# BatsResearch/menghini-neurips23-code

Measured on AMD Instinct MI355X. Metric: images/sec CLIP ViT-B/16 encode+prompt-step, higher is better.
Workload: dtype f16

## Files before the change

menghini-neurips23-code_amd/csrc/attention_split.hip:

```cpp
#include <math.h>

#include "common.h"

__device__ __forceinline__ int vt_index_fwd_s(int key, int d) { return vt_index(key, ((d >> 2) & 3) * 16 + (d >> 4) * 4 + (d & 3)); }

__device__ __forceinline__ void split8(const f32x4 a, const f32x4 b, half8& hi, half8& lo) {
    half4 h0, l0, h1, l1;
    split_f16x4(a, h0, l0);
    split_f16x4(b, h1, l1);
    hi = (half8){h0[0], h0[1], h0[2], h0[3], h1[0], h1[1], h1[2], h1[3]};
    lo = (half8){l0[0], l0[1], l0[2], l0[3], l1[0], l1[1], l1[2], l1[3]};
}

template <int KVC, bool CAUSAL, int NW>
__global__ __launch_bounds__(NW * 64) void attn_fwd_split_kernel(const float* __restrict__ qkv, half_t* __restrict__ out, int S, int H) {
    constexpr int SP = KVC * 32;
    constexpr float LOG2E = 1.4426950408889634f;
    constexpr float INV = 1.0f / (float)GRIP_SPLIT_LO_SCALE;
    extern __shared__ __attribute__((aligned(16))) char smem[];
    half_t* Kh = (half_t*)smem;
    half_t* Kl = Kh + SP * 64;
    half_t* Vh = Kl + SP * 64;
    half_t* Vl = Vh + SP * 64;

    const int tid = threadIdx.x, lane = tid & 63, wave = tid >> 6;
    const int D = H * 64;
    const int b = blockIdx.x / H, h = blockIdx.x - b * H;
    const size_t ld = (size_t)3 * D;
    const float* base = qkv + (size_t)b * S * ld + h * 64;
    const int li = lane & 15, lg = lane >> 4;
    const int n_qt = (S + 15) >> 4;

    for (int idx = tid; idx < SP * 8; idx += NW * 64) {
        const int row = idx >> 3, chunk = idx & 7;
        f32x4 a = {0.f, 0.f, 0.f, 0.f}, c = {0.f, 0.f, 0.f, 0.f};
        if (row < S) {
            const f32x4* p = (const f32x4*)(base + (size_t)row * ld + D + chunk * 8);
            a = p[0];
            c = p[1];
        }
        half8 hi, lo;
        split8(a, c, hi, lo);
        const int o = row * 64 + ((chunk ^ (row & 7)) * 8);
        *(half8*)(Kh + o) = hi;
        *(half8*)(Kl + o) = lo;
    }
    for (int idx = tid; idx < ((SP / 2 + 31) / 32) * 256; idx += NW * 64) {
        const int lane_rp = idx & 31, chunk = ((idx >> 5) & 1) + 2 * ((idx >> 6) & 3), rblk = idx >> 8;
        const int r0 = 2 * (rblk * 32 + lane_rp);
        if (r0 >= SP) continue;
        f32x4 z = {0.f, 0.f, 0.f, 0.f};
        f32x4 a0 = z, a1 = z, b0 = z, b1 = z;
        if (r0 < S) { const f32x4* p = (const f32x4*)(base + (size_t)r0 * ld + 2 * D + chunk * 8); a0 = p[0]; a1 = p[1]; }
        if (r0 + 1 < S) { const f32x4* p = (const f32x4*)(base + (size_t)(r0 + 1) * ld + 2 * D + chunk * 8); b0 = p[0]; b1 = p[1]; }
        half8 h0, l0, h1, l1;
        split8(a0, a1, h0, l0);
        split8(b0, b1, h1, l1);
#pragma unroll
        for (int j = 0; j < 8; ++j) {
            const int o = vt_index_fwd_s(r0, chunk * 8 + j);
            *(half2v*)(Vh + o) = (half2v){h0[j], h1[j]};
            *(half2v*)(Vl + o) = (half2v){l0[j], l1[j]};
        }
    }
    __syncthreads();

    for (int qt = wave; qt < n_qt; qt += NW) {
        asm volatile("" ::: "memory");
        const int qrow = qt * 16 + li;
        const int qr = qrow < S ? qrow : S - 1;
        half8 qh[2], ql[2];
#pragma unroll
        for (int kk = 0; kk < 2; ++kk) {
            const f32x4* p = (const f32x4*)(base + (size_t)qr * ld + (kk * 4 + lg) * 8);
            split8(p[0] * 0.125f, p[1] * 0.125f, qh[kk], ql[kk]);
        }
        f32x4 sc[2 * KVC];
        float m = -INFINITY;
#pragma unroll
        for (int t = 0; t < 2 * KVC; ++t) {
            f32x4 acc = {0.f, 0.f, 0.f, 0.f}, cor = {0.f, 0.f, 0.f, 0.f};
#pragma unroll
            for (int kk = 0; kk < 2; ++kk) {
                const int o = (t * 16 + li) * 64 + (((kk * 4 + lg) ^ (lane & 7)) * 8);
                const half8 kh = *(const half8*)(Kh + o), kl = *(const half8*)(Kl + o);
                acc = __builtin_amdgcn_mfma_f32_16x16x32_f16(kh, qh[kk], acc, 0, 0, 0);
                cor = __builtin_amdgcn_mfma_f32_16x16x32_f16(kl, qh[kk], cor, 0, 0, 0);
                cor = __builtin_amdgcn_mfma_f32_16x16x32_f16(kh, ql[kk], cor, 0, 0, 0);
            }
            acc += cor * INV;
            if (CAUSAL || t >= 2 * (KVC - 1)) {
#pragma unroll
                for (int r = 0; r < 4; ++r) {
                    const int kv = t * 16 + lg * 4 + r;
                    if (kv >= S || (CAUSAL && kv > qrow)) acc[r] = -INFINITY;
                }
            }
            m = fmaxf(fmaxf(fmaxf(m, acc[0]), fmaxf(acc[1], acc[2])), acc[3]);
            sc[t] = acc;
        }
        m = fmaxf(m, __shfl_xor(m, 16));
        m = fmaxf(m, __shfl_xor(m, 32));
        const float m2 = m * LOG2E;
#pragma unroll
        for (int t = 0; t < 2 * KVC; ++t)
#pragma unroll
            for (int r = 0; r < 4; ++r) sc[t][r] = __builtin_amdgcn_exp2f(__builtin_fmaf(sc[t][r], LOG2E, -m2));

        const half8 ones = {1, 1, 1, 1, 1, 1, 1, 1};
        f32x4 sum_h = {0.f, 0.f, 0.f, 0.f}, sum_l = {0.f, 0.f, 0.f, 0.f};
        f32x4 o[4], oc[4];
#pragma unroll
        for (int nf = 0; nf < 4; ++nf) { o[nf] = (f32x4){0.f, 0.f, 0.f, 0.f}; oc[nf] = (f32x4){0.f, 0.f, 0.f, 0.f}; }
#pragma unroll
        for (int c = 0; c < KVC; ++c) {
            half8 ph, pl;
            split8(sc[2 * c], sc[2 * c + 1], ph, pl);
#pragma unroll
            for (int nf = 0; nf < 4; ++nf) {
                const int vo = (c * 4 + nf) * 512 + (lg * 16 + (li ^ lg)) * 8;
                const half8 vh = *(const half8*)(Vh + vo), vl = *(const half8*)(Vl + vo);
                o[nf] = __builtin_amdgcn_mfma_f32_16x16x32_f16(vh, ph, o[nf], 0, 0, 0);
                oc[nf] = __builtin_amdgcn_mfma_f32_16x16x32_f16(vl, ph, oc[nf], 0, 0, 0);
                oc[nf] = __builtin_amdgcn_mfma_f32_16x16x32_f16(vh, pl, oc[nf], 0, 0, 0);
            }
            sum_h = __builtin_amdgcn_mfma_f32_16x16x32_f16(ones, ph, sum_h, 0, 0, 0);
            sum_l = __builtin_amdgcn_mfma_f32_16x16x32_f16(ones, pl, sum_l, 0, 0, 0);
        }
        if (qrow < S) {
            const float inv = 1.0f / (sum_h[0] + sum_l[0] * INV);
            half_t* orow = out + (size_t)((size_t)b * S + qrow) * 2 * D;
            const int col = h * 64 + lg * 16;
            half_t* op = orow + (col >> 5) * 64 + (col & 31);
            half8 hi0, lo0, hi1, lo1;
            split8((o[0] + oc[0] * INV) * inv, (o[1] + oc[1] * INV) * inv, hi0, lo0);
            split8((o[2] + oc[2] * INV) * inv, (o[3] + oc[3] * INV) * inv, hi1, lo1);
            *(half8*)op = hi0;
            *(half8*)(op + 8) = hi1;
            *(half8*)(op + 32) = lo0;
            *(half8*)(op + 40) = lo1;
        }
    }
}

bool attention_split_supported(int S) { return S >= 1 && S <= 320; }

int launch_attention_fwd_split(const float* qkv, void* out, int B, int S, int H, int causal, hipStream_t s) {
    GRIP_REQUIRE(attention_split_supported(S) && B >= 1 && H >= 1, "attention_split: bad shape B=%d S=%d H=%d (S <= 320)", B, S, H);
    const int kvc = (S + 31) / 32;
    const size_t lds = (size_t)4 * kvc * 32 * 64 * sizeof(half_t);
#define GRIP_ATT_CASE(K)                                                                                                                     \
    case K: {                                                                                                                                \
        static bool configured = false;                                                                                                      \
        if (!configured) {                                                                                                                   \
            GRIP_CHECK_HIP(hipFuncSetAttribute((const void*)attn_fwd_split_kernel<K, false, (K >= 4 ? 8 : 4)>, hipFuncAttributeMaxDynamicSharedMemorySize, (int)lds)); \
            GRIP_CHECK_HIP(hipFuncSetAttribute((const void*)attn_fwd_split_kernel<K, true, (K >= 4 ? 8 : 4)>, hipFuncAttributeMaxDynamicSharedMemorySize, (int)lds));  \
            configured = true;                                                                                                               \
        }                                                                                                                                    \
        if (causal) hipLaunchKernelGGL((attn_fwd_split_kernel<K, true, (K >= 4 ? 8 : 4)>), dim3(B * H), dim3((K >= 4 ? 8 : 4) * 64), lds, s, qkv, (half_t*)out, S, H); \
        else hipLaunchKernelGGL((attn_fwd_split_kernel<K, false, (K >= 4 ? 8 : 4)>), dim3(B * H), dim3((K >= 4 ? 8 : 4) * 64), lds, s, qkv, (half_t*)out, S, H);       \
    } break;
    switch (kvc) {
        GRIP_ATT_CASE(1) GRIP_ATT_CASE(2) GRIP_ATT_CASE(3) GRIP_ATT_CASE(4) GRIP_ATT_CASE(5)
        GRIP_ATT_CASE(6) GRIP_ATT_CASE(7) GRIP_ATT_CASE(8) GRIP_ATT_CASE(9) GRIP_ATT_CASE(10)
        default: GRIP_REQUIRE(false, "attention_split: S = %d out of range", S);
    }
#undef GRIP_ATT_CASE
    GRIP_CHECK_HIP(hipGetLastError());
    return GRIP_OK;
}
```

menghini-neurips23-code_amd/csrc/common.h:

```cpp
#pragma once
#include <hip/hip_runtime.h>
#include <stdint.h>
#include <stdio.h>
#include <string.h>

#include "host_common.h"
#include "gemm_plan.h"

typedef _Float16 half_t;
typedef half_t half8 __attribute__((ext_vector_type(8)));
typedef half_t half4 __attribute__((ext_vector_type(4)));
typedef half_t half2v __attribute__((ext_vector_type(2)));
typedef float f32x4 __attribute__((ext_vector_type(4)));

typedef half_t resid_t;

#define AS1 __attribute__((address_space(1)))
#define AS3 __attribute__((address_space(3)))

#define GRIP_CHECK_HIP(expr)                                                                   \
    do {                                                                                       \
        hipError_t _e = (expr);                                                                \
        if (_e != hipSuccess) {                                                                \
            grip_set_error("%s:%d %s -> %s", __FILE__, __LINE__, #expr, hipGetErrorString(_e)); \
// ... 12 lines not shown
}

#define LN_EPS 1e-5f
#define MAX_NV 8

__device__ __forceinline__ float wave_sum(float v) {
#define GRIP_DPP_ADD(ctrl) v += __builtin_bit_cast(float, __builtin_amdgcn_update_dpp(0, __builtin_bit_cast(int, v), ctrl, 0xF, 0xF, true))
    GRIP_DPP_ADD(0xB1);
    GRIP_DPP_ADD(0x4E);
    GRIP_DPP_ADD(0x141);
    GRIP_DPP_ADD(0x140);
#undef GRIP_DPP_ADD
    const int b = __builtin_bit_cast(int, v);
    const float r0 = __builtin_bit_cast(float, __builtin_amdgcn_readlane(b, 0)), r1 = __builtin_bit_cast(float, __builtin_amdgcn_readlane(b, 16));
    const float r2 = __builtin_bit_cast(float, __builtin_amdgcn_readlane(b, 32)), r3 = __builtin_bit_cast(float, __builtin_amdgcn_readlane(b, 48));
    return (r0 + r1) + (r2 + r3);
}
__device__ __forceinline__ float row16_sum(float v) {
#define GRIP_DPP_ADD(ctrl) v += __builtin_bit_cast(float, __builtin_amdgcn_update_dpp(0, __builtin_bit_cast(int, v), ctrl, 0xF, 0xF, true))
    GRIP_DPP_ADD(0xB1);
    GRIP_DPP_ADD(0x4E);
    GRIP_DPP_ADD(0x141);
    GRIP_DPP_ADD(0x140);
#undef GRIP_DPP_ADD
    return v;
}

__device__ __forceinline__ f32x4 load4(const float* p, int i) { return ((const f32x4*)p)[i]; }
__device__ __forceinline__ f32x4 load4(const half_t* p, int i) {
    const half4 h = ((const half4*)p)[i];
    return (f32x4){(float)h[0], (float)h[1], (float)h[2], (float)h[3]};
}
__device__ __forceinline__ void store4(float* p, int i, f32x4 v) { ((f32x4*)p)[i] = v; }
__device__ __forceinline__ void store4(half_t* p, int i, f32x4 v) { ((half4*)p)[i] = (half4){(half_t)v[0], (half_t)v[1], (half_t)v[2], (half_t)v[3]}; }
#ifndef GRIP_SPLIT_LO_SCALE
#define GRIP_SPLIT_LO_SCALE 1
#endif
#define SP1_W_SCALE 256.0f
__device__ __forceinline__ float quick_gelu_exact_s(float x) { return x * __builtin_amdgcn_rcpf(1.0f + __builtin_amdgcn_exp2f(-1.702f * 1.4426950408889634f * x)); }
struct SplitRow { half_t* p; };
__device__ __forceinline__ void split_f16x4(f32x4 v, half4& hi, half4& lo) {
#pragma unroll
    for (int e = 0; e < 4; ++e) {
        float x = v[e];
        asm volatile("" : "+v"(x));
        const half_t h = (half_t)x;
        hi[e] = h;
        lo[e] = (half_t)((x - (float)h) * (float)GRIP_SPLIT_LO_SCALE);
    }
}
__device__ __forceinline__ void store4(SplitRow r, int i, f32x4 v) {
    half4 hi, lo;
    split_f16x4(v, hi, lo);
    half_t* o = r.p + (i >> 3) * 64 + (i & 7) * 4;
    *(half4*)o = hi;
    *(half4*)(o + 32) = lo;
}

template <int NV>
__device__ __forceinline__ void ln_normalize(f32x4 (&v)[NV], int lane, int d4, int d, float& mean, float& rstd) {
#pragma clang fp contract(off)
    float s = 0.f;
#pragma unroll
    for (int i = 0; i < NV; ++i)
        if (lane + 64 * i < d4) s += v[i][0] + v[i][1] + v[i][2] + v[i][3];
    mean = wave_sum(s) / (float)d;
    float q = 0.f;
#pragma unroll
    for (int i = 0; i < NV; ++i)
        if (lane + 64 * i < d4) {
            f32x4 c = v[i] - mean;
            q += c[0] * c[0] + c[1] * c[1] + c[2] * c[2] + c[3] * c[3];
        }
    rstd = rsqrtf(wave_sum(q) / (float)d + LN_EPS);
}
__device__ __forceinline__ f32x4 ln_apply(f32x4 v, float mean, float rstd, f32x4 g, f32x4 b) {
#pragma clang fp contract(off)
    return (v - mean) * rstd * g + b;
}
#endif

struct GemmArgs {
    const void* A;
    const void* W;
    int M, N, K;
    int variant;
    int64_t m_pad;
    const float* bias;
    const void* resid;
    const void* aux;
    void* out;
    void* out2;
    int ldc;
    float scalar;
    int f32;
    float* stat_part;
    const float* rowstat;
    const float* stat_in;
    int stat_parts;
    const float* colsum;
    int ksplit;
    int64_t split_stride;
    float* coop_scratch;
    int* coop_counter;
    int rot_rows;
    half_t* resid_lo;
    int w_exact;
    int ablate;
};

int launch_gemm(int epi, const GemmArgs& a, hipStream_t s);
int launch_gemm_f32(int epi, const GemmArgs& a, hipStream_t s);
int launch_gemm_split(int epi, const GemmArgs& a, hipStream_t s);
int launch_split_rows(const float* x, void* out, int64_t rows, int K, int64_t ld_in, hipStream_t s, int is_weight = 0, int* overflow_flag = nullptr,
                      int* lo_nonzero_flag = nullptr);
float gemm_split_weight_scale();
bool gemm_split_dup_weights();
int launch_split_dup_weights(const void* src, void* dst, int64_t rows, int K, hipStream_t s);
int launch_gemm_split_k64p(int epi, const GemmArgs& a, hipStream_t s);

int launch_im2col(const void* images, int images_f16, void* out, int out_f32, int B, int R, int patch, int Kpad, hipStream_t s);
int launch_vit_assemble_ln(const float* patch_out, const float* cls, const float* pos, const float* prefix, int P,
                           const float* gamma, const float* beta, void* x, int f32, float* rowstat, int B, int G2, int d, hipStream_t s, half_t* x_lo = nullptr,
                           int per_image = 0);
int launch_vit_deep_insert(const float* deep, void* x, int f32, half_t* x_lo, float* stat_part, float* rowstat, int B, int S, int P, int M, int d, hipStream_t s);
int launch_text_deep_insert(const float* deep, int prefix_classes, void* x, int f32, float* stat_part, float* rowstat, int C, int S, int P, int shared_rows, int M, int d,
                            hipStream_t s);
int launch_ln_stats_finalize(const float* stat_part, int parts, float* rowstat, int M, int d, hipStream_t s);
int launch_ln_fold_weights(const half_t* W, const float* gamma, const float* beta, const float* bias, half_t* Wg, float* colsum, float* bias_out,
                           int N, int K, hipStream_t s);
int launch_layernorm_f16(const void* x, const float* gamma, const float* beta, void* out, int f32, int M, int d, hipStream_t s);
int launch_gather_ln_f16(const void* x, const int32_t* row_index, int row_stride, const float* gamma, const float* beta,
                         void* out, int f32, int n_rows, int d, hipStream_t s);
int launch_text_embed(const int32_t* token_ids, int ld_ids, const float* tok_emb, const float* pos, const float* prefix, int P,
                      int prefix_classes, void* x, int f32, float* rowstat, int C, int T, int d, int vocab, hipStream_t s, int shared_rows = 0);
int launch_transpose(const void* in, void* out, int f32, int rows, int cols, int ld_in, hipStream_t s);

#ifdef __HIPCC__
__device__ __forceinline__ size_t seq_row(int b, int r, int S, int Ps) {
    return r < Ps ? (size_t)r : (size_t)Ps + (size_t)b * (S - Ps) + (r - Ps);
}
#endif

int launch_attention_fwd(const half_t* qkv, half_t* out, int B, int S, int H, int causal, hipStream_t s, int shared_rows = 0);
int launch_attention_row(const half_t* qkv, const half_t* qrows, const int32_t* row_index, half_t* out, int B, int S, int H, int causal, hipStream_t s, int train = 0);
int launch_gather_rows(const half_t* x, const int32_t* row_index, int row_stride, half_t* out, int n_rows, int d, hipStream_t s);
int launch_attention_row_bwd(const half_t* qkv, const half_t* o_rows, const half_t* do_rows, const int32_t* row_index, half_t* dqkv, int B, int S, int H, int causal,
                             hipStream_t s);
int launch_attention_fwd_f32(const float* qkv, float* out, int B, int S, int H, int causal, hipStream_t s, int split_out = 0);
int launch_attention_row_f32(const float* qkv, const float* qrows, const int32_t* row_index, float* out, int B, int S, int H, int causal, hipStream_t s, int split_out = 0);
int launch_gather_rows4(const void* x, const int32_t* row_index, int row_stride, void* out, int n_rows, int d, hipStream_t s);
bool attention_split_supported(int S);
int launch_attention_fwd_split(const float* qkv, void* out, int B, int S, int H, int causal, hipStream_t s);
int launch_attention_bwd(const half_t* qkv, const half_t* o, const half_t* d_out, half_t* dqkv, int B, int S, int H, int causal, hipStream_t s,
                         int shared_rows = 0, float* kv_part = nullptr);
int launch_attention_bwd_tiled(const half_t* qkv, const half_t* o, const half_t* d_out, half_t* dqkv, int B, int S, int H, int causal, hipStream_t s);
int launch_layernorm_f16_from_f32(const float* x, const float* gamma, const float* beta, half_t* out, int M, int d, hipStream_t s);
int launch_ln_bwd_add(const resid_t* x, const float* dln, int parts, int64_t part_stride, const float* gamma, float* dx, half_t* dxh, int M, int d, hipStream_t s);
int launch_ln_bwd_init(const resid_t* x, const float* dln, int parts, int64_t part_stride, const float* gamma, const float* rows_add, const int32_t* index, int stride,
                       float* dx, half_t* dxh, int M, int d, hipStream_t s);
int launch_ln_bwd_scatter(const resid_t* x, const float* dy, const int32_t* index, int stride, const float* gamma, float* dx, half_t* dxh,
                          int n, int d, hipStream_t s);
int launch_ln_bwd_scatter_fill(const resid_t* x, const float* dy, const int32_t* index, int stride, int first, const float* gamma, float* dx, half_t* dxh,
                               int n, int M, int d, hipStream_t s);
int launch_vit_prefix_grad(const float* dx, const float* prefix, const float* gamma, const float* scale, float* grad, int B, int S, int P, int d, hipStream_t s);
int launch_vit_deep_grad(float* dx, half_t* dxh, const float* scale, float* grad, int B, int S, int P, int d, hipStream_t s);
int launch_vit_prefix_grad_per_image(const float* dx, const float* prefix, const float* gamma, const float* scale, float* grad, int B, int S, int P, int d, hipStream_t s);
int launch_text_prefix_grad(const float* dx, const float* scale, float* grad, int C, int T, int P, int prefix_classes, int d, hipStream_t s);
int launch_text_deep_grad(float* dx, half_t* dxh, const float* scale, float* grad, int C, int T, int P, int prefix_classes, int d, hipStream_t s);
int launch_grad_scale_cast(const float* g, half_t* g16, float* scale, int n, hipStream_t s);
```

menghini-neurips23-code_amd/csrc/tower.hip:

```cpp
#include <stdarg.h>
#include <stdlib.h>

#include <map>
#include <string>
#include <vector>

#include "common.h"

static thread_local char g_err[512] = "";
void grip_set_error(const char* fmt, ...) {
    va_list ap;
    va_start(ap, fmt);
    vsnprintf(g_err, sizeof(g_err), fmt, ap);
    va_end(ap);
}
extern "C" const char* grip_last_error(void) { return g_err; }
extern "C" int grip_abi_version(void) { return GRIP_ABI_VERSION; }

static int g_cu_budget = 0;
int grip_cu_budget() { return g_cu_budget; }
extern "C" int grip_set_cu_budget(int n_cus) {
    GRIP_REQUIRE(n_cus >= 0 && (n_cus == 0 || n_cus >= 8), "set_cu_budget: %d (0 = all, else at least 8)", n_cus);
    g_cu_budget = n_cus;
    return GRIP_OK;
// ... 630 lines not shown
extern "C" int grip_text_forward_deep(grip_tower* t, const int32_t* token_ids, const int32_t* eot_index, const float* prefix,
                                      int n_prefix, int prefix_classes, const float* deep, int n_deep, int n_class, int seq_len, float* out_emb,
                                      void* workspace, size_t workspace_bytes, int flags, uint64_t* generation, void* stream) {
    try {
        GRIP_REQUIRE(t && t->D.kind == 1, "text_forward: not a text tower%s", n_deep ? " (the vision tower's deep prompts go through grip_vit_forward_deep)" : "");
        GRIP_REQUIRE(n_deep >= 0 && n_deep <= t->D.layers - 1, "text_forward_deep: n_deep = %d out of range: deep prompts replace the context rows entering blocks 1 .. n_deep, "
                     "0 <= n_deep <= layers - 1 = %d", n_deep, t->D.layers - 1);
        GRIP_REQUIRE(n_deep == 0 || n_prefix > 0, "text_forward_deep: deep prompts replace the rows of the shallow context: n_prefix must be positive (n_deep = %d)", n_deep);
        GRIP_REQUIRE(n_deep == 0 || deep, "text_forward_deep: null deep prompt pointer (n_deep = %d)", n_deep);
        GRIP_REQUIRE(token_ids && eot_index && out_emb && (n_prefix == 0 || prefix), "text_forward: null pointer");
        GRIP_REQUIRE(!(flags & GRIP_FWD_PER_IMAGE_PREFIX), "text_forward: GRIP_FWD_PER_IMAGE_PREFIX is a vision-tower flag (one context per class: prefix_classes = n_class)");
        GRIP_REQUIRE(n_prefix == 0 || prefix_classes == 1 || prefix_classes == n_class, "text_forward: prefix_classes must be 1 or n_class");
        GRIP_REQUIRE((flags & ~(GRIP_FWD_TRAIN | GRIP_FWD_SHARED_PREFIX | GRIP_FWD_NO_POS_EMB)) == 0, "text_forward: unknown flag bits 0x%x", flags);
        const int train = flags & GRIP_FWD_TRAIN;
        const int shared = (flags & GRIP_FWD_SHARED_PREFIX) && n_prefix > 0 && prefix_classes == 1 && !t->f32;
        Workspace w;
        RUN(check_ws(t, n_class, n_prefix, train, workspace, workspace_bytes, w, seq_len, shared));
        w.deep = n_deep ? deep : nullptr;
        w.n_deep = n_deep;
        w.deep_classes = n_deep ? prefix_classes : 1;
        hipStream_t s = (hipStream_t)stream;
        const grip_dims& D = t->D;
        const int d = D.width, f = t->f32;
        const float* F = t->w32;
        resid_t* x0 = train ? w.x_in[0] : w.x;
        if (train && w.coop_cnt) GRIP_CHECK_HIP(hipMemsetAsync(w.coop_cnt, 0, w.coop_cnt_bytes, s));
        RUN(launch_text_embed(token_ids, D.seq0, F + t->L.tok, (flags & GRIP_FWD_NO_POS_EMB) ? nullptr : F + t->L.pos, prefix, n_prefix, prefix_classes, x0, f, (train && !train_fold(t)) ? nullptr : w.rowstat, n_class, w.S, d, D.vocab, s, w.Ps));
        resid_t* xf = nullptr;
        bool compact = false;
        RUN(run_blocks(t, w, x0, 1, eot_index, s, &xf, &compact));
        RUN(launch_gather_ln_f16(xf, compact ? nullptr : eot_index, compact ? 1 : w.rs, F + t->L.lnpost_g, F + t->L.lnpost_b, w.cls16, f, n_class, d, s));
        GemmArgs a{};
        a.f32 = f; a.A = w.cls16; a.W = t->wop(t->L.projT); a.M = n_class; a.N = D.embed_dim; a.K = d; a.out = out_emb; a.ldc = D.embed_dim;
        RUN(launch_gemm(EPI_F32, a, s));
        note_forward(t, workspace, train, w, eot_index, prefix_classes, generation, false, n_deep);
        return GRIP_OK;
    } catch (...) { grip_set_error("text_forward: exception"); return GRIP_ERR_ARG; }
}

extern "C" int grip_text_forward(grip_tower* t, const int32_t* token_ids, const int32_t* eot_index, const float* prefix,
                                 int n_prefix, int prefix_classes, int n_class, int seq_len, float* out_emb,
                                 void* workspace, size_t workspace_bytes, int flags, uint64_t* generation, void* stream) {
    return grip_text_forward_deep(t, token_ids, eot_index, prefix, n_prefix, prefix_classes, nullptr, 0, n_class, seq_len, out_emb, workspace, workspace_bytes, flags,
                                  generation, stream);
}

extern "C" int grip_debug_gemm(int epi, const void* A, const void* W, int M, int N, int K, const float* bias, const void* resid,
                               const void* aux, void* out, void* out2, float scalar, int m_pad, int variant, void* stream) {
    GemmArgs a{};
    a.variant = variant & 0xff;
    a.rot_rows = (variant >> 8) & 1;
    a.A = A; a.W = W; a.M = M; a.N = N; a.K = K; a.m_pad = m_pad; a.bias = bias; a.resid = resid;
    a.aux = aux; a.out = out; a.out2 = out2; a.ldc = N; a.scalar = scalar;
    if (a.variant == 7) { a.f32 = 1; a.variant = 0; }
    return launch_gemm(epi, a, (hipStream_t)stream);
}
extern "C" int grip_debug_gemm_splitk(const void* A, const void* W, int M, int N, int K, float* out, int ksplit, int64_t split_stride, int* ksplit_used,
                                      int m_pad, int variant, void* stream) {
    GemmArgs a{};
    a.variant = variant & 0xff;
    a.rot_rows = (variant >> 8) & 1;
    a.A = A; a.W = W; a.M = M; a.N = N; a.K = K; a.m_pad = m_pad; a.out = out; a.ldc = N;
    a.ksplit = ksplit ? ksplit : gemm_pick_ksplit(M, N, K);
    a.split_stride = split_stride;
    if (ksplit_used) *ksplit_used = a.ksplit;
    return launch_gemm(EPI_F32, a, (hipStream_t)stream);
}
extern "C" int grip_debug_gemm_ln(int epi, const void* A, const void* W, int M, int N, int K, const float* bias, const void* resid, void* out, void* out2,
                                  float* stat_part, const float* rowstat, const float* colsum, int m_pad, int variant, void* stream) {
    GemmArgs a{};
    a.variant = variant;
    a.A = A; a.W = W; a.M = M; a.N = N; a.K = K; a.m_pad = m_pad; a.bias = bias; a.resid = resid; a.out = out; a.out2 = out2; a.ldc = N;
    a.stat_part = stat_part; a.rowstat = rowstat; a.colsum = colsum;
    return launch_gemm(epi, a, (hipStream_t)stream);
}
extern "C" int grip_debug_gemm_train(int epi, const void* A, const void* W, int M, int N, int K, const float* bias, const void* resid, void* out, void* out2,
                                     float* stat_part, float* rowstat, const float* colsum, const float* stat_in, int stat_parts, int ksplit,
                                     float* coop_scratch, int* coop_counter, int m_pad, void* stream) {
    GemmArgs a{};
    a.rot_rows = 1;
    a.A = A; a.W = W; a.M = M; a.N = N; a.K = K; a.m_pad = m_pad; a.bias = bias; a.resid = resid; a.out = out; a.out2 = out2; a.ldc = N;
    a.stat_part = stat_part; a.rowstat = rowstat; a.colsum = colsum; a.stat_in = stat_in; a.stat_parts = stat_parts;
    a.ksplit = ksplit; a.coop_scratch = coop_scratch; a.coop_counter = coop_counter;
    return launch_gemm(epi, a, (hipStream_t)stream);
}
extern "C" int grip_debug_gemm_args(int epi, const void* A, const void* W, int M, int N, int K, int ldc, const float* bias, const void* resid, void* resid_lo,
                                    const void* aux, void* out, void* out2, float scalar, float* stat_part, float* rowstat, const float* colsum,
                                    const float* stat_in, int stat_parts, int ksplit, int64_t split_stride, float* coop_scratch, int* coop_counter, int m_pad,
                                    int variant, int rot_rows, void* stream) {
    GemmArgs a{};
    a.A = A; a.W = W; a.M = M; a.N = N; a.K = K; a.ldc = ldc; a.m_pad = m_pad; a.variant = variant; a.rot_rows = rot_rows;
    a.bias = bias; a.resid = resid; a.resid_lo = (half_t*)resid_lo; a.aux = aux; a.out = out; a.out2 = out2; a.scalar = scalar;
    a.stat_part = stat_part; a.rowstat = rowstat; a.colsum = colsum; a.stat_in = stat_in; a.stat_parts = stat_parts;
    a.ksplit = ksplit; a.split_stride = split_stride; a.coop_scratch = coop_scratch; a.coop_counter = coop_counter;
    return launch_gemm(epi, a, (hipStream_t)stream);
}
extern "C" int grip_debug_coop_split(int M, int N, int K) { return gemm_pick_coop_split(M, N, K); }
extern "C" int grip_debug_ln_fold(const void* W, const float* gamma, const float* beta, const float* bias, void* Wg, float* colsum, float* bias_out,
                                  int N, int K, const float* stat_part, int parts, float* rowstat, int M, int d, void* stream) {
    int rc = W ? launch_ln_fold_weights((const half_t*)W, gamma, beta, bias, (half_t*)Wg, colsum, bias_out, N, K, (hipStream_t)stream) : GRIP_OK;
    if (rc || !stat_part) return rc;
    return launch_ln_stats_finalize(stat_part, parts, rowstat, M, d, (hipStream_t)stream);
}
extern "C" int grip_debug_gemm_split(int epi, const float* A, const float* W, int M, int N, int K, const float* bias, const float* resid, void* out,
                                     void* a_split, void* w_split, int m_pad, void* stream) {
    hipStream_t s = (hipStream_t)stream;
    RUN(launch_split_rows(A, a_split, m_pad, K, K, s));
    int* flag = nullptr;
    GRIP_CHECK_HIP(hipMalloc((void**)&flag, sizeof(int)));
    int inexact = 1;
    int rc = hipMemsetAsync(flag, 0, sizeof(int), s) == hipSuccess ? launch_split_rows(W, w_split, N, K, K, s, 1, nullptr, flag) : GRIP_ERR_HIP;
    if (!rc && (hipMemcpyAsync(&inexact, flag, sizeof(int), hipMemcpyDeviceToHost, s) != hipSuccess || hipStreamSynchronize(s) != hipSuccess)) rc = GRIP_ERR_HIP;
    (void)hipFree(flag);
    if (rc) return rc;
    GemmArgs a{};
    a.w_exact = !inexact && gemm_split_dup_weights();
    a.f32 = 2; a.A = a_split; a.W = w_split; a.M = M; a.N = N; a.K = K; a.m_pad = m_pad; a.bias = bias; a.resid = resid; a.out = out; a.ldc = N;
    if (!a.w_exact) return launch_gemm(epi, a, s);
    void* w_dup = nullptr;
    GRIP_CHECK_HIP(hipMalloc(&w_dup, (size_t)N * K * 4));
    a.W = w_dup;
    rc = launch_split_dup_weights(w_split, w_dup, N, K, s);
    if (!rc) rc = launch_gemm(epi, a, s);
    if (hipStreamSynchronize(s) != hipSuccess && !rc) { grip_set_error("debug_gemm_split: HIP error"); rc = GRIP_ERR_HIP; }
    (void)hipFree(w_dup);
    return rc;
}
int gemm_split_last_wlo();
extern "C" int grip_debug_split_last_wlo(void) { return gemm_split_last_wlo(); }
extern "C" int grip_debug_split_rows(const float* x, void* out, int64_t rows, int K, void* stream) {
    return launch_split_rows(x, out, rows, K, K, (hipStream_t)stream);
}
extern "C" int grip_debug_gemm_tier(int tier, int w_exact, int epi, const void* A, const void* W, int M, int N, int K, int ldc, const float* bias, const void* resid,
                                    void* out, void* out2, float scalar, int64_t m_pad, void* stream) {
    GemmArgs a{};
    a.f32 = tier; a.w_exact = w_exact;
    a.A = A; a.W = W; a.M = M; a.N = N; a.K = K; a.ldc = ldc; a.m_pad = m_pad; a.bias = bias; a.resid = resid; a.out = out; a.out2 = out2; a.scalar = scalar;
    return launch_gemm(epi, a, (hipStream_t)stream);
}
extern "C" int grip_debug_split_weights(const float* W, void* image, int64_t rows, int K, int dup, int* flags_out, void* stream) {
    hipStream_t s = (hipStream_t)stream;
    int* flag = nullptr;
    GRIP_CHECK_HIP(hipMalloc((void**)&flag, 2 * sizeof(int)));
    int rc = hipMemsetAsync(flag, 0, 2 * sizeof(int), s) == hipSuccess ? launch_split_rows(W, image, rows, K, K, s, 1, flag, flag + 1) : GRIP_ERR_HIP;
    if (!rc && dup) rc = launch_split_dup_weights(image, image, rows, K, s);
    if (!rc && (hipMemcpyAsync(flags_out, flag, 2 * sizeof(int), hipMemcpyDeviceToHost, s) != hipSuccess || hipStreamSynchronize(s) != hipSuccess)) {
        grip_set_error("debug_split_weights: HIP error");
        rc = GRIP_ERR_HIP;
    }
    (void)hipFree(flag);
    return rc;
}
extern "C" int grip_debug_attention_split(const void* qkv, void* out, int B, int S, int H, int causal, int mfma, void* stream) {
    if (mfma) return launch_attention_fwd_split((const float*)qkv, out, B, S, H, causal, (hipStream_t)stream);
    return launch_attention_fwd_f32((const float*)qkv, (float*)out, B, S, H, causal, (hipStream_t)stream, 1);
}
extern "C" int grip_debug_attention_exact(const void* qkv, void* out, int B, int S, int H, int causal, void* stream) {
    return launch_attention_fwd_f32((const float*)qkv, (float*)out, B, S, H, causal, (hipStream_t)stream);
}
extern "C" int grip_debug_attention(const void* qkv, void* out, int B, int S, int H, int causal, void* stream) {
    return launch_attention_fwd((const half_t*)qkv, (half_t*)out, B, S, H, causal, (hipStream_t)stream);
}
extern "C" int grip_debug_attention_shared(const void* qkv, void* out, int B, int S, int H, int shared_rows, void* stream) {
    return launch_attention_fwd((const half_t*)qkv, (half_t*)out, B, S, H, 1, (hipStream_t)stream, shared_rows);
}
extern "C" int grip_debug_attention_row(const void* qkv, const void* qrows, const int32_t* row_index, void* out, int B, int S, int H, int causal, int train,
                                        void* stream) {
    return launch_attention_row((const half_t*)qkv, (const half_t*)qrows, row_index, (half_t*)out, B, S, H, causal, (hipStream_t)stream, train);
}
extern "C" int grip_debug_attention_row_exact(const void* qkv, const void* qrows, const int32_t* row_index, void* out, int B, int S, int H, int causal,
                                              int split_out, void* stream) {
    return launch_attention_row_f32((const float*)qkv, (const float*)qrows, row_index, (float*)out, B, S, H, causal, (hipStream_t)stream, split_out);
}
extern "C" int grip_debug_layernorm(const float* x, const float* gamma, const float* beta, void* out, int M, int d, void* stream) {
    return launch_layernorm_f16_from_f32(x, gamma, beta, (half_t*)out, M, d, (hipStream_t)stream);
}
extern "C" int grip_debug_ln_bwd_add(const void* x, const float* dln, int parts, int64_t part_stride, const float* gamma, float* dx, void* dxh, int M, int d,
                                     void* stream) {
    return launch_ln_bwd_add((const resid_t*)x, dln, parts, part_stride, gamma, dx, (half_t*)dxh, M, d, (hipStream_t)stream);
}
extern "C" int grip_debug_ln_bwd_init(const void* x, const float* dln, int parts, int64_t part_stride, const float* gamma, const float* rows_add,
                                      const int32_t* index, int stride, float* dx, void* dxh, int M, int d, void* stream) {
    return launch_ln_bwd_init((const resid_t*)x, dln, parts, part_stride, gamma, rows_add, index, stride, dx, (half_t*)dxh, M, d, (hipStream_t)stream);
}
extern "C" int grip_debug_ln_bwd_scatter(const void* x, const float* dy, const int32_t* index, int stride, int first, const float* gamma, float* dx, void* dxh,
                                         int n, int M, int d, int fill, void* stream) {
    if (fill) return launch_ln_bwd_scatter_fill((const resid_t*)x, dy, index, stride, first, gamma, dx, (half_t*)dxh, n, M, d, (hipStream_t)stream);
    return launch_ln_bwd_scatter((const resid_t*)x, dy, index, stride, gamma, dx, (half_t*)dxh, n, d, (hipStream_t)stream);
}
extern "C" int grip_debug_vit_prefix_grad(float* dx, void* dxh, const float* prefix, const float* gamma, const float* scale, float* grad, int B, int S, int P,
                                          int d, int mode, void* stream) {
    if (mode == 0) return launch_vit_prefix_grad(dx, prefix, gamma, scale, grad, B, S, P, d, (hipStream_t)stream);
    if (mode == 1) return launch_vit_prefix_grad_per_image(dx, prefix, gamma, scale, grad, B, S, P, d, (hipStream_t)stream);
    return launch_vit_deep_grad(dx, (half_t*)dxh, scale, grad, B, S, P, d, (hipStream_t)stream);
}
extern "C" int grip_debug_text_prefix_grad(float* dx, void* dxh, const float* scale, float* grad, int C, int T, int P, int prefix_classes, int d, int deep,
                                           void* stream) {
    if (deep) return launch_text_deep_grad(dx, (half_t*)dxh, scale, grad, C, T, P, prefix_classes, d, (hipStream_t)stream);
    return launch_text_prefix_grad(dx, scale, grad, C, T, P, prefix_classes, d, (hipStream_t)stream);
}
extern "C" int grip_debug_grad_scale_cast(const float* g, void* g16, float* scale, int n, void* stream) {
    return launch_grad_scale_cast(g, (half_t*)g16, scale, n, (hipStream_t)stream);
}
extern "C" int grip_debug_layernorm_modes(const void* x, const int32_t* row_index, int row_stride, const float* gamma, const float* beta, void* out, int f32,
                                          int gather, int M, int d, void* stream) {
    if (gather) return launch_gather_ln_f16(x, row_index, row_stride, gamma, beta, out, f32, M, d, (hipStream_t)stream);
    return launch_layernorm_f16(x, gamma, beta, out, f32, M, d, (hipStream_t)stream);
}
extern "C" int grip_debug_vit_assemble(const float* patch_out, const float* cls, const float* pos, const float* prefix, int P, const float* gamma, const float* beta,
                                       void* x, int f32, float* rowstat, int B, int G2, int d, void* x_lo, int per_image, void* stream) {
    return launch_vit_assemble_ln(patch_out, cls, pos, prefix, P, gamma, beta, x, f32, rowstat, B, G2, d, (hipStream_t)stream, (half_t*)x_lo, per_image);
}
extern "C" int grip_debug_deep_insert(const float* deep, int prefix_classes, void* x, int f32, void* x_lo, float* stat_part, float* rowstat, int B, int S, int P,
                                      int shared_rows, int M, int d, int text, void* stream) {
    if (text) return launch_text_deep_insert(deep, prefix_classes, x, f32, stat_part, rowstat, B, S, P, shared_rows, M, d, (hipStream_t)stream);
    return launch_vit_deep_insert(deep, x, f32, (half_t*)x_lo, stat_part, rowstat, B, S, P, M, d, (hipStream_t)stream);
}
extern "C" int grip_debug_text_embed(const int32_t* ids, int ld_ids, const float* tok_emb, const float* pos, const float* prefix, int P, int prefix_classes, void* x,
                                     int f32, float* rowstat, int C, int T, int d, int vocab, int shared_rows, void* stream) {
    return launch_text_embed(ids, ld_ids, tok_emb, pos, prefix, P, prefix_classes, x, f32, rowstat, C, T, d, vocab, (hipStream_t)stream, shared_rows);
}
extern "C" int grip_debug_patch_gather(const void* images, int images_f16, void* out, int out_f32, int B, int R, int patch, int Kpad, void* stream) {
    return launch_im2col(images, images_f16, out, out_f32, B, R, patch, Kpad, (hipStream_t)stream);
}
extern "C" int grip_debug_transpose(const void* in, void* out, int f32, int rows, int cols, int ld_in, void* stream) {
    return launch_transpose(in, out, f32, rows, cols, ld_in, (hipStream_t)stream);
}
extern "C" int grip_debug_gather_rows(const void* x, const int32_t* row_index, int row_stride, void* out, int n_rows, int d, int four_byte, void* stream) {
    if (four_byte) return launch_gather_rows4(x, row_index, row_stride, out, n_rows, d, (hipStream_t)stream);
    return launch_gather_rows((const half_t*)x, row_index, row_stride, (half_t*)out, n_rows, d, (hipStream_t)stream);
}

static int run_blocks_backward(grip_tower* t, Workspace& w, int causal, const int32_t* read_rows, hipStream_t s, float* grad_deep = nullptr) {
    const int d = t->D.width, H = t->D.heads;
    const half_t* W = t->w16;
    const float* F = t->w32;
    const int64_t part = (int64_t)w.Mp * d;
    for (int l = t->D.layers - 1; l >= 0; --l) {
        const LayerW& lw = t->L.layer[(size_t)l];
        if (grad_deep && l + 1 <= w.n_deep) {
            if (t->D.kind == 0)
                RUN(launch_vit_deep_grad(w.dx, w.dxh, w.scale, grad_deep + (size_t)l * w.P * d, w.batch, w.S, w.P, d, s));
            else
                RUN(launch_text_deep_grad(w.dx, w.dxh, w.scale, grad_deep + (size_t)l * w.deep_classes * w.P * d, w.Ps ? 1 : w.batch, w.S, w.P, w.deep_classes, d, s));
        }
        if (l + 1 == t->D.layers && w.rows_last) {
            const int64_t Bp = round_up64(w.batch, 256);
            const int64_t rpart = Bp * d;
            GemmArgs a{};
            a.A = w.drow_h; a.W = W + lw.proj_wT; a.M = w.batch; a.m_pad = Bp; a.N = 4 * d; a.K = d; a.aux = w.row_hpre; a.out = w.row_dh; a.ldc = 4 * d;
            RUN(launch_gemm(EPI_GELUGRAD_F16, a, s));
            a = GemmArgs{};
            a.A = w.row_dh; a.W = W + lw.fc_wT; a.M = w.batch; a.m_pad = Bp; a.N = d; a.K = 4 * d; a.out = w.row_dln; a.ldc = d;
            a.ksplit = w.ks_row; a.split_stride = rpart;
            RUN(launch_gemm(EPI_F32, a, s));
            RUN(launch_ln_bwd_add(w.row_xmid, w.row_dln, w.ks_row, rpart, F + lw.ln2_g, w.drow, w.drow_h, w.batch, d, s));
            a = GemmArgs{};
            a.A = w.drow_h; a.W = W + lw.out_wT; a.M = w.batch; a.m_pad = Bp; a.N = d; a.K = d; a.out = w.row_datt; a.ldc = d;
            RUN(launch_gemm(EPI_F16, a, s));
            RUN(launch_attention_row_bwd(w.qkv_l[(size_t)l], w.row_att, w.row_datt, read_rows, w.dqkv, w.batch, w.S, H, causal, s));
            a = GemmArgs{};
            a.rot_rows = 1;
            a.A = w.dqkv; a.W = W + lw.in_wT; a.M = w.M; a.m_pad = w.Mp; a.N = d; a.K = 3 * d; a.out = w.dln; a.ldc = d;
            a.ksplit = w.ks_in; a.split_stride = part;
            RUN(launch_gemm(EPI_F32, a, s));
            RUN(launch_ln_bwd_init(w.x_in[(size_t)l], w.dln, w.ks_in, part, F + lw.ln1_g, w.drow, read_rows, w.S, w.dx, w.dxh, w.M, d, s));
            continue;
        }
        GemmArgs a{};
        a.rot_rows = 1;
        a.A = w.dxh; a.W = W + lw.proj_wT; a.M = w.M; a.m_pad = w.Mp; a.N = 4 * d; a.K = d; a.aux = w.hpre_l[(size_t)l]; a.out = w.dh; a.ldc = 4 * d;
        RUN(launch_gemm(EPI_GELUGRAD_F16, a, s));
        a = GemmArgs{};
        a.rot_rows = 1;
        a.A = w.dh; a.W = W + lw.fc_wT; a.M = w.M; a.m_pad = w.Mp; a.N = d; a.K = 4 * d; a.out = w.dln; a.ldc = d;
        a.ksplit = w.ks_fc; a.split_stride = part;
        RUN(launch_gemm(EPI_F32, a, s));
        RUN(launch_ln_bwd_add(w.x_mid[(size_t)l], w.dln, w.ks_fc, part, F + lw.ln2_g, w.dx, w.dxh, w.M, d, s));
        a = GemmArgs{};
        a.rot_rows = 1;
        a.A = w.dxh; a.W = W + lw.out_wT; a.M = w.M; a.m_pad = w.Mp; a.N = d; a.K = d; a.out = w.datt; a.ldc = d;
        RUN(launch_gemm(EPI_F16, a, s));
        RUN(launch_attention_bwd(w.qkv_l[(size_t)l], w.att_l[(size_t)l], w.datt, w.dqkv, w.batch, w.S, H, causal, s, w.Ps, w.kv_part));
        a = GemmArgs{};
        a.rot_rows = 1;
        a.A = w.dqkv; a.W = W + lw.in_wT; a.M = w.M; a.m_pad = w.Mp; a.N = d; a.K = 3 * d; a.out = w.dln; a.ldc = d;
        a.ksplit = w.ks_in; a.split_stride = part;
        RUN(launch_gemm(EPI_F32, a, s));
        RUN(launch_ln_bwd_add(w.x_in[(size_t)l], w.dln, w.ks_in, part, F + lw.ln1_g, w.dx, w.dxh, w.M, d, s));
    }
    return GRIP_OK;
}

static int backward_head_of_tower(grip_tower* t, Workspace& w, const float* grad_emb, const int32_t* index, hipStream_t s) {
    const grip_dims& D = t->D;
    const int d = D.width;
    RUN(launch_grad_scale_cast(grad_emb, w.gemb16, w.scale, w.batch * D.embed_dim, s));
    GemmArgs a{};
    a.A = w.gemb16; a.W = t->w16 + t->L.proj; a.M = w.batch; a.N = d; a.K = D.embed_dim; a.out = w.dcls; a.ldc = d;
    RUN(launch_gemm(EPI_F32, a, s));
    if (w.rows_last)
        return launch_ln_bwd_scatter(w.row_xout, w.dcls, nullptr, 1, t->w32 + t->L.lnpost_g, w.drow, w.drow_h, w.batch, d, s);
    RUN(launch_ln_bwd_scatter_fill(w.x_in[(size_t)D.layers], w.dcls, index, w.rs, w.Ps, t->w32 + t->L.lnpost_g, w.dx, w.dxh, w.batch, (int)w.M, d, s));
    return GRIP_OK;
}

// ... 125 lines not shown
```

Measured before the change: 21100.

## Batch global loads via buffer intrinsics and prefetch next Q tile in split attention

Adds a new split-precision attention forward kernel. It issues every K/V global load into registers up front using raw buffer loads, where out-of-bounds offsets return zero, and only then splits the values and writes them to LDS. This lets the memory requests overlap instead of going one loop iteration at a time. It also prefetches the next query tile while the current one is computed, and hoists the LDS base offsets out of the loop. The old kernel stays available as a reference through an env var and a debug entry point, at the cost of more registers held across the staging phase.

```diff
diff --git a/menghini-neurips23-code_amd/csrc/attention_split.hip b/menghini-neurips23-code_amd/csrc/attention_split.hip
--- a/menghini-neurips23-code_amd/csrc/attention_split.hip
+++ b/menghini-neurips23-code_amd/csrc/attention_split.hip
@@ -1,4 +1,5 @@
 #include <math.h>
+#include <stdlib.h>
 
 #include "common.h"
 
@@ -13,7 +14,7 @@
 }
 
 template <int KVC, bool CAUSAL, int NW>
-__global__ __launch_bounds__(NW * 64) void attn_fwd_split_kernel(const float* __restrict__ qkv, half_t* __restrict__ out, int S, int H) {
+__global__ __launch_bounds__(NW * 64) void attn_fwd_split_ref_kernel(const float* __restrict__ qkv, half_t* __restrict__ out, int S, int H) {
     constexpr int SP = KVC * 32;
     constexpr float LOG2E = 1.4426950408889634f;
     constexpr float INV = 1.0f / (float)GRIP_SPLIT_LO_SCALE;
@@ -143,29 +144,206 @@
     }
 }
 
+template <int KVC, bool CAUSAL, int NW>
+__global__ __launch_bounds__(NW * 64) void attn_fwd_split_kernel(const float* __restrict__ qkv, half_t* __restrict__ out, int S, int H) {
+    constexpr int SP = KVC * 32;
+    constexpr float LOG2E = 1.4426950408889634f;
+    constexpr float INV = 1.0f / (float)GRIP_SPLIT_LO_SCALE;
+    constexpr int NT = NW * 64;
+    constexpr int KTOT = SP * 8, KT = (KTOT + NT - 1) / NT;
+    constexpr int VTOT = ((SP / 2 + 31) / 32) * 256, VT = (VTOT + NT - 1) / NT;
+    extern __shared__ __attribute__((aligned(16))) char smem[];
+    half_t* Kh = (half_t*)smem;
+    half_t* Kl = Kh + SP * 64;
+    half_t* Vh = Kl + SP * 64;
+    half_t* Vl = Vh + SP * 64;
+
+    const int tid = threadIdx.x, lane = tid & 63, wave = tid >> 6;
+    const int D = H * 64;
+    const int b = blockIdx.x / H, h = blockIdx.x - b * H;
+    const int li = lane & 15, lg = lane >> 4;
+    const int n_qt = (S + 15) >> 4;
+    const uint32_t ldb = (uint32_t)(3 * D) * 4u, seq_bytes = (uint32_t)S * ldb;
+    const __amdgpu_buffer_rsrc_t seq = __builtin_amdgcn_make_buffer_rsrc((void*)(qkv + (size_t)b * S * 3 * D), 0, (int)seq_bytes, 0x00020000);
+    auto load8 = [&](bool pred, int row, int col, f32x4& x, f32x4& y) {
+        const uint32_t off = pred ? (uint32_t)row * ldb + (uint32_t)(h * 64 + col) * 4u : seq_bytes;
+        x = __builtin_bit_cast(f32x4, __builtin_amdgcn_raw_buffer_load_b128(seq, (int)off, 0, 0));
+        y = __builtin_bit_cast(f32x4, __builtin_amdgcn_raw_buffer_load_b128(seq, (int)(off + 16u), 0, 0));
+    };
+    auto load_q = [&](int qt, f32x4 (&q)[4]) {
+        const int qrow = qt * 16 + li;
+        const int qr = qrow < S ? qrow : S - 1;
+#pragma unroll
+        for (int kk = 0; kk < 2; ++kk) load8(true, qr, (kk * 4 + lg) * 8, q[2 * kk], q[2 * kk + 1]);
+    };
+
+    f32x4 ka[KT], kc[KT];
+#pragma unroll
+    for (int t = 0; t < KT; ++t) {
+        const int idx = tid + t * NT, row = idx >> 3, chunk = idx & 7;
+        load8(idx < KTOT && row < S, row, D + chunk * 8, ka[t], kc[t]);
+    }
+    f32x4 va0[VT], va1[VT], vb0[VT], vb1[VT];
+#pragma unroll
+    for (int t = 0; t < VT; ++t) {
+        const int idx = tid + t * NT;
+        const int lane_rp = idx & 31, chunk = ((idx >> 5) & 1) + 2 * ((idx >> 6) & 3), rblk = idx >> 8;
+        const int r0 = 2 * (rblk * 32 + lane_rp);
+        const bool mine = idx < VTOT && r0 < SP;
+        load8(mine && r0 < S, r0, 2 * D + chunk * 8, va0[t], va1[t]);
+        load8(mine && r0 + 1 < S, r0 + 1, 2 * D + chunk * 8, vb0[t], vb1[t]);
+    }
+    f32x4 q[4];
+    load_q(wave < n_qt ? wave : 0, q);
+
+#pragma unroll
+    for (int t = 0; t < KT; ++t) {
+        const int idx = tid + t * NT, row = idx >> 3, chunk = idx & 7;
+        if (idx < KTOT) {
+            half8 hi, lo;
+            split8(ka[t], kc[t], hi, lo);
+            const int o = row * 64 + ((chunk ^ (row & 7)) * 8);
+            *(half8*)(Kh + o) = hi;
+            *(half8*)(Kl + o) = lo;
+        }
+    }
+#pragma unroll
+    for (int t = 0; t < VT; ++t) {
+        const int idx = tid + t * NT;
+        const int lane_rp = idx & 31, chunk = ((idx >> 5) & 1) + 2 * ((idx >> 6) & 3), rblk = idx >> 8;
+        const int r0 = 2 * (rblk * 32 + lane_rp);
+        if (idx < VTOT && r0 < SP) {
+            half8 h0, l0, h1, l1;
+            split8(va0[t], va1[t], h0, l0);
+            split8(vb0[t], vb1[t], h1, l1);
+#pragma unroll
+            for (int j = 0; j < 8; ++j) {
+                const int o = vt_index_fwd_s(r0, chunk * 8 + j);
+                *(half2v*)(Vh + o) = (half2v){h0[j], h1[j]};
+                *(half2v*)(Vl + o) = (half2v){l0[j], l1[j]};
+            }
+        }
+    }
+    __syncthreads();
+
+    int kho[2] = {li * 64 + ((lg ^ (lane & 7)) * 8), li * 64 + (((4 + lg) ^ (lane & 7)) * 8)};
+    int klo[2] = {kho[0] + SP * 64, kho[1] + SP * 64};
+    int vho = 2 * SP * 64 + (lg * 16 + (li ^ lg)) * 8, vlo = vho + SP * 64;
+    asm volatile("" : "+v"(kho[0]), "+v"(kho[1]), "+v"(klo[0]), "+v"(klo[1]), "+v"(vho), "+v"(vlo));
+    for (int qt = wave; qt < n_qt; qt += NW) {
+        asm volatile("" ::: "memory");
+        const int qrow = qt * 16 + li;
+        half8 qh[2], ql[2];
+#pragma unroll
+        for (int kk = 0; kk < 2; ++kk) split8(q[2 * kk] * 0.125f, q[2 * kk + 1] * 0.125f, qh[kk], ql[kk]);
+        if (qt + NW < n_qt) load_q(qt + NW, q);
+        f32x4 sc[2 * KVC];
+        float m = -INFINITY;
+#pragma unroll
+        for (int t = 0; t < 2 * KVC; ++t) {
+            f32x4 acc = {0.f, 0.f, 0.f, 0.f}, cor = {0.f, 0.f, 0.f, 0.f};
+#pragma unroll
+            for (int kk = 0; kk < 2; ++kk) {
+                const half8 kh = *(const half8*)(Kh + kho[kk] + t * 1024), kl = *(const half8*)(Kh + klo[kk] + t * 1024);
+                acc = __builtin_amdgcn_mfma_f32_16x16x32_f16(kh, qh[kk], acc, 0, 0, 0);
+                cor = __builtin_amdgcn_mfma_f32_16x16x32_f16(kl, qh[kk], cor, 0, 0, 0);
+                cor = __builtin_amdgcn_mfma_f32_16x16x32_f16(kh, ql[kk], cor, 0, 0, 0);
+            }
+            acc += cor * INV;
+            if (CAUSAL || t >= 2 * (KVC - 1)) {
+#pragma unroll
+                for (int r = 0; r < 4; ++r) {
+                    const int kv = t * 16 + lg * 4 + r;
+                    if (kv >= S || (CAUSAL && kv > qrow)) acc[r] = -INFINITY;
+                }
+            }
+            m = fmaxf(fmaxf(fmaxf(m, acc[0]), fmaxf(acc[1], acc[2])), acc[3]);
+            sc[t] = acc;
+        }
+        m = fmaxf(m, __shfl_xor(m, 16));
+        m = fmaxf(m, __shfl_xor(m, 32));
+        const float m2 = m * LOG2E;
+#pragma unroll
+        for (int t = 0; t < 2 * KVC; ++t)
+#pragma unroll
+            for (int r = 0; r < 4; ++r) sc[t][r] = __builtin_amdgcn_exp2f(__builtin_fmaf(sc[t][r], LOG2E, -m2));
+
+        const half8 ones = {1, 1, 1, 1, 1, 1, 1, 1};
+        f32x4 sum_h = {0.f, 0.f, 0.f, 0.f}, sum_l = {0.f, 0.f, 0.f, 0.f};
+        f32x4 o[4], oc[4];
+#pragma unroll
+        for (int nf = 0; nf < 4; ++nf) { o[nf] = (f32x4){0.f, 0.f, 0.f, 0.f}; oc[nf] = (f32x4){0.f, 0.f, 0.f, 0.f}; }
+#pragma unroll
+        for (int c = 0; c < KVC; ++c) {
+            half8 ph, pl;
+            split8(sc[2 * c], sc[2 * c + 1], ph, pl);
+#pragma unroll
+            for (int nf = 0; nf < 4; ++nf) {
+                const half8 vh = *(const half8*)(Kh + vho + (c * 4 + nf) * 512), vl = *(const half8*)(Kh + vlo + (c * 4 + nf) * 512);
+                o[nf] = __builtin_amdgcn_mfma_f32_16x16x32_f16(vh, ph, o[nf], 0, 0, 0);
+                oc[nf] = __builtin_amdgcn_mfma_f32_16x16x32_f16(vl, ph, oc[nf], 0, 0, 0);
+                oc[nf] = __builtin_amdgcn_mfma_f32_16x16x32_f16(vh, pl, oc[nf], 0, 0, 0);
+            }
+            sum_h = __builtin_amdgcn_mfma_f32_16x16x32_f16(ones, ph, sum_h, 0, 0, 0);
+            sum_l = __builtin_amdgcn_mfma_f32_16x16x32_f16(ones, pl, sum_l, 0, 0, 0);
+        }
+        if (qrow < S) {
+            const float inv = 1.0f / (sum_h[0] + sum_l[0] * INV);
+            half_t* orow = out + (size_t)((size_t)b * S + qrow) * 2 * D;
+            const int col = h * 64 + lg * 16;
+            half_t* op = orow + (col >> 5) * 64 + (col & 31);
+            half8 hi0, lo0, hi1, lo1;
+            split8((o[0] + oc[0] * INV) * inv, (o[1] + oc[1] * INV) * inv, hi0, lo0);
+            split8((o[2] + oc[2] * INV) * inv, (o[3] + oc[3] * INV) * inv, hi1, lo1);
+            *(half8*)op = hi0;
+            *(half8*)(op + 8) = hi1;
+            *(half8*)(op + 32) = lo0;
+            *(half8*)(op + 40) = lo1;
+        }
+    }
+}
+
 bool attention_split_supported(int S) { return S >= 1 && S <= 320; }
 
-int launch_attention_fwd_split(const float* qkv, void* out, int B, int S, int H, int causal, hipStream_t s) {
+static int launch_attention_fwd_split_form(const float* qkv, void* out, int B, int S, int H, int causal, int form, hipStream_t s) {
     GRIP_REQUIRE(attention_split_supported(S) && B >= 1 && H >= 1, "attention_split: bad shape B=%d S=%d H=%d (S <= 320)", B, S, H);
     const int kvc = (S + 31) / 32;
     const size_t lds = (size_t)4 * kvc * 32 * 64 * sizeof(half_t);
-#define GRIP_ATT_CASE(K)                                                                                                                     \
-    case K: {                                                                                                                                \
+#define GRIP_ATT_LAUNCH(KERNEL, K, C)                                                                                                        \
+    do {                                                                                                                                     \
         static bool configured = false;                                                                                                      \
         if (!configured) {                                                                                                                   \
-            GRIP_CHECK_HIP(hipFuncSetAttribute((const void*)attn_fwd_split_kernel<K, false, (K >= 4 ? 8 : 4)>, hipFuncAttributeMaxDynamicSharedMemorySize, (int)lds)); \
-            GRIP_CHECK_HIP(hipFuncSetAttribute((const void*)attn_fwd_split_kernel<K, true, (K >= 4 ? 8 : 4)>, hipFuncAttributeMaxDynamicSharedMemorySize, (int)lds));  \
+            GRIP_CHECK_HIP(hipFuncSetAttribute((const void*)KERNEL<K, C, (K >= 4 ? 8 : 4)>, hipFuncAttributeMaxDynamicSharedMemorySize, (int)lds)); \
             configured = true;                                                                                                               \
         }                                                                                                                                    \
-        if (causal) hipLaunchKernelGGL((attn_fwd_split_kernel<K, true, (K >= 4 ? 8 : 4)>), dim3(B * H), dim3((K >= 4 ? 8 : 4) * 64), lds, s, qkv, (half_t*)out, S, H); \
-        else hipLaunchKernelGGL((attn_fwd_split_kernel<K, false, (K >= 4 ? 8 : 4)>), dim3(B * H), dim3((K >= 4 ? 8 : 4) * 64), lds, s, qkv, (half_t*)out, S, H);       \
-    } break;
+        hipLaunchKernelGGL((KERNEL<K, C, (K >= 4 ? 8 : 4)>), dim3(B * H), dim3((K >= 4 ? 8 : 4) * 64), lds, s, qkv, (half_t*)out, S, H);          \
+    } while (0)
+#define GRIP_ATT_CASE(K)                                                                                                                     \
+    case K:                                                                                                                                  \
+        if (form) {                                                                                                                          \
+            if (causal) GRIP_ATT_LAUNCH(attn_fwd_split_kernel, K, true);                                                                     \
+            else GRIP_ATT_LAUNCH(attn_fwd_split_kernel, K, false);                                                                           \
+        } else {                                                                                                                             \
+            if (causal) GRIP_ATT_LAUNCH(attn_fwd_split_ref_kernel, K, true);                                                                 \
+            else GRIP_ATT_LAUNCH(attn_fwd_split_ref_kernel, K, false);                                                                       \
+        }                                                                                                                                    \
+        break;
     switch (kvc) {
         GRIP_ATT_CASE(1) GRIP_ATT_CASE(2) GRIP_ATT_CASE(3) GRIP_ATT_CASE(4) GRIP_ATT_CASE(5)
         GRIP_ATT_CASE(6) GRIP_ATT_CASE(7) GRIP_ATT_CASE(8) GRIP_ATT_CASE(9) GRIP_ATT_CASE(10)
         default: GRIP_REQUIRE(false, "attention_split: S = %d out of range", S);
     }
 #undef GRIP_ATT_CASE
+#undef GRIP_ATT_LAUNCH
     GRIP_CHECK_HIP(hipGetLastError());
     return GRIP_OK;
 }
+
+int launch_attention_fwd_split(const float* qkv, void* out, int B, int S, int H, int causal, hipStream_t s) {
+    static const bool ref = getenv("GRIP_ATTN_SPLIT_FORM") && atoi(getenv("GRIP_ATTN_SPLIT_FORM")) == 0;
+    return launch_attention_fwd_split_form(qkv, out, B, S, H, causal, ref ? 0 : 1, s);
+}
+
+int launch_attention_fwd_split_ref(const float* qkv, void* out, int B, int S, int H, int causal, hipStream_t s) {
+    return launch_attention_fwd_split_form(qkv, out, B, S, H, causal, 0, s);
+}
diff --git a/menghini-neurips23-code_amd/csrc/common.h b/menghini-neurips23-code_amd/csrc/common.h
--- a/menghini-neurips23-code_amd/csrc/common.h
+++ b/menghini-neurips23-code_amd/csrc/common.h
@@ -188,6 +188,7 @@
 int launch_gather_rows4(const void* x, const int32_t* row_index, int row_stride, void* out, int n_rows, int d, hipStream_t s);
 bool attention_split_supported(int S);
 int launch_attention_fwd_split(const float* qkv, void* out, int B, int S, int H, int causal, hipStream_t s);
+int launch_attention_fwd_split_ref(const float* qkv, void* out, int B, int S, int H, int causal, hipStream_t s);
 int launch_attention_bwd(const half_t* qkv, const half_t* o, const half_t* d_out, half_t* dqkv, int B, int S, int H, int causal, hipStream_t s,
                          int shared_rows = 0, float* kv_part = nullptr);
 int launch_attention_bwd_tiled(const half_t* qkv, const half_t* o, const half_t* d_out, half_t* dqkv, int B, int S, int H, int causal, hipStream_t s);
diff --git a/menghini-neurips23-code_amd/csrc/tower.hip b/menghini-neurips23-code_amd/csrc/tower.hip
--- a/menghini-neurips23-code_amd/csrc/tower.hip
+++ b/menghini-neurips23-code_amd/csrc/tower.hip
@@ -806,6 +806,7 @@
     return rc;
 }
 extern "C" int grip_debug_attention_split(const void* qkv, void* out, int B, int S, int H, int causal, int mfma, void* stream) {
+    if (mfma == 2) return launch_attention_fwd_split_ref((const float*)qkv, out, B, S, H, causal, (hipStream_t)stream);
     if (mfma) return launch_attention_fwd_split((const float*)qkv, out, B, S, H, causal, (hipStream_t)stream);
     return launch_attention_fwd_f32((const float*)qkv, (float*)out, B, S, H, causal, (hipStream_t)stream, 1);
 }
```

Measured after the change: 21190 (median of 6 runs). About the same (+0.4%).
